# biotite-dev/springcraft

Hardware: AMD Instinct MI355X
Metric: ANM modes/sec (Hessian build + full eigensolve), N=2000 C-alpha (higher is better)
Workload: dtype f64; 1 GPU; C3: N=2000 C-alpha ANM, HinsenForceField (no cutoff), full 6000x6000 eigensolve, all modes + vectors; parallelism=independent structures sharded over GPUs, no data-path collective

## Files before the change

### include/springcraft_hip_debug.h

```cpp
#ifndef SPRINGCRAFT_HIP_DEBUG_H
#define SPRINGCRAFT_HIP_DEBUG_H

#include "springcraft_hip.h"

#ifdef __cplusplus
extern "C" {
#endif

int sc_dbg_gemm_bench(sc_ctx* ctx, int m, int n, int k, int mode, int tile, int split_k, int iters, int beta_one,
                      double* ms_out, double* max_err_out);

int sc_dbg_gemm_host(sc_ctx* ctx, const double* a, const double* b, double* c, int m, int n, int k, int mode, int tile,
                     int split_k, double alpha, double beta, int lower_grid);

int sc_dbg_gemm3_host(sc_ctx* ctx, const double* a, const double* b, double* c, int count, int m, int n, int k, int layout,
                      int lower, double beta);

int sc_dbg_symm3_host(sc_ctx* ctx, const double* a, const double* v, double* x, int count, int m, int split);
int sc_dbg_symm3_stamps(unsigned long long* out4);
int sc_dbg_symm3_bench(sc_ctx* ctx, int count, int m, int split, int iters, double* ms_out);

int sc_dbg_gemm3_bench(sc_ctx* ctx, int count, int m, int n, int k, int layout, int lower, int kernel, int order, int iters,
                       double* ms_out);

int sc_dbg_gemm_stamps(unsigned long long* out4, int reset);

int sc_dbg_gemm_trace(unsigned long long* out, int max_records, int* count, int reset);

int sc_dbg_two_stage(sc_ctx* ctx, const double* a, int n, double* band_out, double* d_out, double* e_out);

int sc_dbg_bt2_stamps(unsigned long long* out);

int sc_dbg_bt2_clock(unsigned long long* out2);

int sc_dbg_bt2_trace(unsigned long long* out);

int sc_dbg_bulge_stamps(unsigned long long* out6);
int sc_dbg_pair_stamps(unsigned long long* out48);
int sc_dbg_chase_stamps(unsigned long long* out16);

int sc_dbg_set_chase(sc_ctx* ctx, int mode, int give_up_after);

int sc_dbg_set_panel_coop(sc_ctx* ctx, int min_rows);
int sc_dbg_set_panel_coop_fail(sc_ctx* ctx, int panel);

int sc_dbg_set_resident(sc_ctx* ctx, int mode, int hook, int workgroups);
// ... 7 lines not shown
```

### springcraft_amd/csrc/gemm_f64.h

```cpp
#pragma once

#include <cstdint>

#include "common.h"

struct GemmDesc {
  const double* a;
  const double* b;
  double* c;
  int m, n, k;
  long long sa_i, sa_k;
  long long sb_k, sb_j;
  long long ldc;
  double alpha, beta;
  const int* a_kidx;
  const int* b_kidx;
  const int* c_jidx;
  int lower_only;
  int row_off, col_off;
  long long split_stride;
  int a_tri;
};

constexpr int kGemmTile = 3;

constexpr int kGemmAmBk = 0, kGemmAkBk = 1, kGemmAmBn = 2;
int launch_gemm_f64(sc_ctx* ctx, const GemmDesc* d_desc, int count, int max_m, int max_n, int tile,
                    int split_k = 1, bool gather = false, bool tri = false, int layout = -1, bool lower_grid = false,
                    int pin_tile = 0);
int gemm_f64_tile(const sc_ctx* ctx, int count, int max_m, int max_n, int layout);

int launch_gemm3_uniform(sc_ctx* ctx, const GemmDesc* d_desc, int count, int m, int n, int k, int layout, int lower,
                         double alpha, double beta, bool aligned16);
bool gemm3_would_take(sc_ctx* ctx, int count, int m, int n, int k, int layout, int lower, double alpha, double beta,
                      bool aligned16);

int launch_symm3(sc_ctx* ctx, const GemmDesc* d_desc, int count, int m, int split, bool aligned16, bool any_size = false);
bool symm3_would_take(sc_ctx* ctx, int count, int m, int split, bool aligned16);
```

### springcraft_amd/csrc/gemm_f64.hip

```cpp
#include <algorithm>
#include <cmath>
#include <cstdlib>
#include <vector>

#include "gemm_f64.h"

namespace {

typedef double d4 __attribute__((ext_vector_type(4)));

template <int X, bool XCONTIG>
struct StageImage {
  static constexpr int kSize = XCONTIG ? 16 * (X + 16) : 8 * (X + 1) * 2;
  __device__ static __forceinline__ int at(int x, int k) {
    return XCONTIG ? k * (X + 16) + x : ((k >> 1) * (X + 1) + x) * 2 + (k & 1);
  }
};

#ifdef GEMM_STAMPS
__device__ unsigned long long g_gemm_stamps[8];
constexpr int kTraceMax = 1 << 16;
__device__ unsigned long long g_gemm_trace[6 * kTraceMax];
__device__ unsigned int g_gemm_trace_n;
#define GEMM_STAMP(var) unsigned long long var; asm volatile("s_memtime %0\n\ts_waitcnt lgkmcnt(0)" : "=s"(var)::"memory");
// ... 231 lines not shown

  GEMM_STAMP(t_loop)
  int buf = 0;
  for (int kt = k_begin; kt < k_end; kt += BK) {
    if (kt + BK < k_end) s_write(buf ^ 1, kt + BK);
    if (kt + 2 * BK < k_end) g_load(kt + 2 * BK);
    const double* a_s = sA + buf * ImgA::kSize + ImgA::at(wm * WM + fr, fk);
    const double* b_s = sB + buf * ImgB::kSize + ImgB::at(wn * WN + fr, fk);
    double af[2][MT], bf[2][NT];
#pragma unroll
    for (int mi = 0; mi < MT; ++mi) af[0][mi] = a_s[ImgA::at(mi * 16, 0)];
#pragma unroll
    for (int ni = 0; ni < NT; ++ni) bf[0][ni] = b_s[ImgB::at(ni * 16, 0)];
#pragma unroll
    for (int k4 = 0; k4 < BK / 4; ++k4) {
      const int cur = k4 & 1, nxt = cur ^ 1;
      if (k4 + 1 < BK / 4) {
#pragma unroll
        for (int mi = 0; mi < MT; ++mi) af[nxt][mi] = a_s[ImgA::at(mi * 16, (k4 + 1) * 4)];
#pragma unroll
        for (int ni = 0; ni < NT; ++ni) bf[nxt][ni] = b_s[ImgB::at(ni * 16, (k4 + 1) * 4)];
      }
#pragma unroll
      for (int ni = 0; ni < NT; ++ni)
#pragma unroll
        for (int mi = 0; mi < MT; ++mi)
          acc[ni][mi] = __builtin_amdgcn_mfma_f64_16x16x4f64(bf[cur][ni], af[cur][mi], acc[ni][mi], 0, 0, 0);
    }
    __syncthreads();
    buf ^= 1;
  }

  GEMM_STAMP(t_epi)
#pragma unroll
  for (int ni = 0; ni < NT; ++ni) {
#pragma unroll
    for (int r = 0; r < 4; ++r) {
      const int col = n0 + wn * WN + ni * 16 + fk + 4 * r;
      if (col >= N) continue;
      gptr ccol = C + (long long)((GATHER && D.c_jidx) ? D.c_jidx[col] : col) * ldc;
#pragma unroll
      for (int mi = 0; mi < MT; ++mi) {
        const int row = m0 + wm * WM + mi * 16 + fr;
        if (row >= M) continue;
        if (lower && (lower2 ? ((row + roff) | 1) : (row + roff)) < (col + coff)) continue;
        ccol[row] = alpha * acc[ni][mi][r];
      }
    }
  }
#ifdef GEMM_STAMPS
  {
    GEMM_STAMP(t_end)
    if (lane == 0) {
      atomicAdd(&g_gemm_stamps[0], t_loop - t_start);
      atomicAdd(&g_gemm_stamps[1], t_epi - t_loop);
      atomicAdd(&g_gemm_stamps[2], t_end - t_epi);
      atomicAdd(&g_gemm_stamps[3], 1ull);
    }
    if (tid == 0) {
      const unsigned slot = atomicAdd(&g_gemm_trace_n, 1u);
      if (slot < (unsigned)kTraceMax) {
        unsigned hwid, xcc;
        asm volatile("s_getreg_b32 %0, hwreg(HW_REG_HW_ID)" : "=s"(hwid));
        asm volatile("s_getreg_b32 %0, hwreg(HW_REG_XCC_ID)" : "=s"(xcc));
        unsigned long long* r = g_gemm_trace + 6ull * slot;
        r[0] = ((unsigned long long)xcc << 32) | hwid;
        r[1] = t_start; r[2] = t_loop; r[3] = t_epi; r[4] = t_end;
        r[5] = blockIdx.x + (unsigned long long)gridDim.x * (blockIdx.y + (unsigned long long)gridDim.y * blockIdx.z);
      }
    }
  }
#endif
}

template <int BM, int BN, bool AM, bool BNC, bool TRI, bool GATHER = false>
void launch_gemm2_inst(hipStream_t st, dim3 grid, const GemmDesc* d_desc, int split_k, bool lower = false) {
  constexpr size_t lds = sizeof(double) * 2 * (size_t)(StageImage<BM, AM>::kSize + StageImage<BN, BNC>::kSize);
  (void)sc_raise_dyn_lds(reinterpret_cast<const void*>(&k_gemm2<BM, BN, AM, BNC, TRI, GATHER>), (int)lds);
  if (lower) {
// ... 225 lines not shown
  D.alpha = alpha; D.beta = beta;
  if (mode == 0) { D.sa_i = 1; D.sa_k = m; D.sb_k = 1; D.sb_j = k; }
  if (mode == 1) { D.sa_i = 1; D.sa_k = m; D.sb_k = n; D.sb_j = 1; D.lower_only = 1; }
  if (mode == 2) { D.sa_i = k; D.sa_k = 1; D.sb_k = 1; D.sb_j = k; }
  D.split_stride = (long long)m * n;
  fail(hipMemcpy(dd, &D, sizeof(D), hipMemcpyHostToDevice));
  if (rc == SC_OK) {
    const int layout = mode == 0 ? kGemmAmBk : (mode == 1 ? kGemmAmBn : kGemmAkBk);
    if (tile < 10 || tile > 13) {
      rc = sc_set_error(ctx, SC_ERR_INVALID_ARG, "tile id %d (10 .. 13)", tile);
    } else {
      g_gemm2_force_tile = tile - 10;
      rc = launch_gemm_f64(ctx, dd, 1, m, n, tile, split_k, false, false, layout, lower_grid != 0);
      g_gemm2_force_tile = 0;
    }
    fail(hipStreamSynchronize(st));
  }
  if (rc == SC_OK) {
    std::vector<double> h(ec);
    fail(hipMemcpy(h.data(), dc, ec * 8, hipMemcpyDeviceToHost));
    if (rc == SC_OK) {
      if (split_k == 1) std::copy(h.begin(), h.end(), c);
      else
        for (size_t i = 0; i < (size_t)m * n; ++i) {
          double sum = 0.0;
          for (int sl = 0; sl < split_k; ++sl) sum += h[(size_t)sl * m * n + i];
          c[i] = sum;
        }
    }
  }
  (void)hipFree(base);
  return rc;
}
```

### springcraft_amd/csrc/sy2sb.hip

```cpp
#include <algorithm>
#include <vector>

#include "twostage_internal.h"

namespace {

constexpr int kEarly = (kIb + 2) / 2;

__global__ __launch_bounds__(256) void k_panel_qr(double* __restrict__ a_all, long long stride_a,
                                                  double* __restrict__ tri_all, TriLayout TL,
                                                  double* __restrict__ sb_all, SbLayout SL, int j0, int j, int nr,
                                                  int c_end) {
  constexpr int LD = kQrRows + 1;
  extern __shared__ __attribute__((aligned(16))) double sm[];
  const int c_lo = j > 0 ? j - 1 : 0;
  const int ncl = c_end - c_lo;
  double* P = sm;
  double* wv = sm + ncl * LD;
  double* vv = wv + kB;
  double* red = vv + kQrRows;
  __shared__ double s_scale, s_beta, s_tau;

  const int n = TL.n;
  const int r0 = j0 + kB, m = n - r0;
// ... 890 lines not shown
      }
      __syncthreads();
    }
    const double tau = s_tau, scale = s_scale;
    for (int c0 = j + 1; c0 < kB; c0 += 8) {
      const int cnt = min(8, kB - c0);
      double a[8] = {0, 0, 0, 0, 0, 0, 0, 0};
      for (int r = j + 1 + tid; r < m; r += 1024) {
        const double x = pj[r];
        for (int i = 0; i < cnt; ++i) a[i] += x * P[(size_t)(c0 + i) * n + r];
      }
      block_sum8(a, cnt);
      if (tid < cnt) s_w[tid] = tau * (P[(size_t)(c0 + tid) * n + j] + scale * a[tid]);
      __syncthreads();
      for (int r = j + tid; r < m; r += 1024) {
        const double v = r > j ? scale * pj[r] : 1.0;
        for (int i = 0; i < cnt; ++i) P[(size_t)(c0 + i) * n + r] -= v * s_w[i];
      }
      __syncthreads();
    }
    for (int r = j + tid; r < m; r += 1024) pj[r] = r > j ? scale * pj[r] : s_beta;
    __syncthreads();
  }
  for (int c = 0; c < kB; ++c)
    for (int r = tid; r < m; r += 1024) {
      const double val = P[(size_t)c * n + r];
      const double v = r > c ? val : (r == c ? 1.0 : 0.0);
      sb[SL.vw + (size_t)c * n + r0 + r] = v;
      sb[SL.wv + (size_t)(kB + c) * n + r0 + r] = -v;
      sb[SL.xv + (size_t)(2 * kB + c) * n + r0 + r] = v;
    }
}

__global__ __launch_bounds__(256) void k_sum_xslices(double* __restrict__ sb_all, SbLayout SL, int r0) {
  const int n = SL.n, p = SL.symm_split;
  double* sb = sb_all + (size_t)blockIdx.z * SL.slab;
  const int which = blockIdx.y / kB, c = blockIdx.y % kB;
  const int r = r0 + blockIdx.x * 256 + threadIdx.x;
  if (r >= n) return;
  const double* src = sb + SL.xsplit + (size_t)which * p * n * kB + (size_t)c * n + r;
  double s = 0.0;
  for (int q = 0; q < p; ++q) s += src[(size_t)q * n * kB];
  sb[SL.xv + (size_t)(which * kB + c) * n + r] = s;
}

__global__ __launch_bounds__(256) void k_sum_p2(double* __restrict__ sb_all, SbLayout SL) {
  double* sb = sb_all + (size_t)blockIdx.y * SL.slab;
  const int i = blockIdx.x * 256 + threadIdx.x;
  double acc = 0.0;
#pragma unroll
  for (int sl = 0; sl < kSmallSplit; ++sl) acc += sb[SL.small2 + (size_t)sl * 2 * kB * kB + i];
  sb[SL.p2 + i] = acc;
}

__global__ __launch_bounds__(1024) void k_sb_small(const double* __restrict__ tri_all, TriLayout TL,
                                                   double* __restrict__ sb_all, SbLayout SL, int j0) {
  constexpr int LD = kB + 1;
  extern __shared__ __attribute__((aligned(16))) double sm[];
  double* G = sm;
  double* M1 = G + kB * LD;
  double* T = M1 + kB * LD;
  double* U = T + kB * LD;
  const double* tri = tri_all + (size_t)blockIdx.x * TL.slab;
  double* sb = sb_all + (size_t)blockIdx.x * SL.slab;
  const int tid = threadIdx.x, nthr = blockDim.x;
  const double* prod = sb + SL.small;
  const size_t slice = (size_t)kB * 3 * kB;
  for (int idx = tid; idx < kB * kB; idx += nthr) {
    const int i = idx & 63, jj = idx >> 6;
    double g = 0.0, x = 0.0;
#pragma unroll
    for (int s = 0; s < kSmallSplit; ++s) {
      const double* ps = prod + s * slice;
      x += ps[i + (size_t)jj * kB] + ps[i + (size_t)(kB + jj) * kB];
      g += ps[i + (size_t)(2 * kB + jj) * kB];
    }
    G[i * LD + jj] = g;
    M1[i * LD + jj] = x;
    T[i * LD + jj] = 0.0;
  }
  __syncthreads();
  if (tid < kB) {
    const int bb = tid >> 4, c = tid & 15, o = bb * 16;
    double x[16];
#pragma unroll
    for (int i = 15; i >= 0; --i) {
      double acc = (i == c) ? 1.0 : 0.0;
#pragma unroll
      for (int l = i + 1; l < 16; ++l) acc -= G[(o + i) * LD + o + l] * x[l];
      x[i] = i <= c ? tri[TL.tau + j0 + o + i] * acc : 0.0;
    }
#pragma unroll
    for (int i = 0; i < 16; ++i) T[(o + i) * LD + o + c] = x[i];
  }
  __syncthreads();
#pragma unroll
  for (int bs = 16; bs <= 32; bs *= 2) {
    const int npair = kB / (2 * bs);
    for (int idx = tid; idx < npair * bs * bs; idx += nthr) {
      const int pr = idx / (bs * bs), e = idx % (bs * bs), i = e / bs, jj = e % bs;
      const int o1 = pr * 2 * bs, o2 = o1 + bs;
      double acc = 0.0;
      for (int l = 0; l <= jj; ++l) acc += G[(o1 + i) * LD + o2 + l] * T[(o2 + l) * LD + o2 + jj];
      U[(o1 + i) * LD + o2 + jj] = acc;
    }
    __syncthreads();
    for (int idx = tid; idx < npair * bs * bs; idx += nthr) {
      const int pr = idx / (bs * bs), e = idx % (bs * bs), i = e / bs, jj = e % bs;
      const int o1 = pr * 2 * bs, o2 = o1 + bs;
      double acc = 0.0;
      for (int l = i; l < bs; ++l) acc += T[(o1 + i) * LD + o1 + l] * U[(o1 + l) * LD + o2 + jj];
      T[(o1 + i) * LD + o2 + jj] = -acc;
    }
    __syncthreads();
  }
  for (int idx = tid; idx < kB * kB; idx += nthr) {
    const int i = idx >> 6, jj = idx & 63;
    double s = 0.0;
    for (int l = 0; l <= jj; ++l) s += M1[i * LD + l] * T[l * LD + jj];
    U[i * LD + jj] = s;
  }
  __syncthreads();
  double* cm = sb + SL.cmat;
  for (int idx = tid; idx < kB * kB; idx += nthr) {
    const int i = idx & 63, jj = idx >> 6;
    double s = 0.0;
    for (int l = 0; l <= i; ++l) s += T[l * LD + i] * U[l * LD + jj];
    const double t = T[i * LD + jj];
    cm[i + (size_t)jj * 3 * kB] = t;
    cm[kB + i + (size_t)jj * 3 * kB] = t;
    cm[2 * kB + i + (size_t)jj * 3 * kB] = -0.5 * s;
  }
}

}


std::vector<GemmDesc> sb_stage1_records(int n, int batch, const std::vector<int>& role, double* d_a, long long stride_a,
                                        double* d_sb_ws, const SbLayout& SL) {
  const sc_host::TwoStageEnv& E = sc_host::two_stage_env();
  const int npanels = (int)role.size();
  std::vector<GemmDesc> h((size_t)npanels * kDescKinds * batch);
  for (int p = 0; p < npanels; ++p) {
    const int j0 = p * kB, r0 = j0 + kB, m = n - r0;
    const int rl = role[(size_t)p];
    const long long vw_w = rl == 2 ? 3 * kB : kB, wv_w = rl == 2 ? 2 * kB : 0;
    for (int b = 0; b < batch; ++b) {
      double* A = d_a + (size_t)b * stride_a;
      double* sb = d_sb_ws + (size_t)b * SL.slab;
      double* a22 = A + (size_t)r0 * n + r0;
      GemmDesc* g = &h[((size_t)p * batch + b) * kDescKinds];
      GemmDesc X1{};
      X1.a = a22; X1.sa_i = 1; X1.sa_k = n; X1.a_tri = 1;
      X1.b = sb + SL.xv + (size_t)2 * kB * n + r0; X1.sb_k = 1; X1.sb_j = n;
      X1.c = sb + SL.xv + r0; X1.ldc = n;
      X1.m = m; X1.n = kB; X1.k = m; X1.alpha = 1.0; X1.beta = 0.0;
      if (SL.symm_split > 1) {
        X1.c = sb + SL.xsplit + r0;
        X1.split_stride = (long long)n * kB;
      }
      g[0] = X1;
      GemmDesc X2 = X1;
      X2.sa_i = n; X2.sa_k = 1; X2.a_tri = 2;
      X2.c = sb + SL.xv + (size_t)kB * n + r0;
      if (SL.symm_split > 1) X2.c = sb + SL.xsplit + (size_t)SL.symm_split * n * kB + r0;
      g[1] = X2;
      GemmDesc P{};
      P.a = sb + SL.xv + (size_t)2 * kB * n + r0; P.sa_i = n; P.sa_k = 1;
      P.b = sb + SL.xv + r0; P.sb_k = 1; P.sb_j = n;
      P.c = sb + SL.small; P.ldc = kB;
      P.m = kB; P.n = 3 * kB; P.k = m; P.alpha = 1.0; P.beta = 0.0;
      P.split_stride = (long long)kB * 3 * kB;
      g[2] = P;
      GemmDesc W{};
      W.a = sb + SL.xv + r0; W.sa_i = 1; W.sa_k = n;
      W.b = sb + SL.cmat; W.sb_k = 1; W.sb_j = 3 * kB;
      W.c = sb + SL.vw + (size_t)vw_w * n + r0; W.ldc = n;
      W.m = m; W.n = kB; W.k = 3 * kB; W.alpha = 1.0; W.beta = 0.0;
      g[3] = W;
      W.c = sb + SL.wv + (size_t)wv_w * n + r0;
      W.alpha = -1.0;
      g[4] = W;
      GemmDesc R{};
      R.a = sb + SL.vw + r0; R.sa_i = 1; R.sa_k = n;
      R.b = sb + SL.wv + r0; R.sb_k = n; R.sb_j = 1;
      R.c = a22; R.ldc = n;
      R.m = m; R.n = m; R.k = rl == 2 ? 4 * kB : 2 * kB; R.alpha = 1.0; R.beta = 1.0;
      R.lower_only = sc_host::symm3_for(E, n) ? 2 : 1;
      g[5] = R;
      GemmDesc D = R;
      D.n = kB; D.k = 2 * kB;
      g[6] = D;
      GemmDesc Q{};
      Q.a = sb + SL.wv + r0; Q.sa_i = n; Q.sa_k = 1;
      Q.b = sb + SL.xv + (size_t)2 * kB * n + r0; Q.sb_k = 1; Q.sb_j = n;
      Q.c = sb + SL.small2; Q.ldc = 2 * kB;
      Q.m = 2 * kB; Q.n = kB; Q.k = m; Q.alpha = 1.0; Q.beta = 0.0;
      Q.split_stride = (long long)2 * kB * kB;
      g[7] = Q;
      GemmDesc Cr{};
      Cr.a = sb + SL.vw + r0; Cr.sa_i = 1; Cr.sa_k = n;
      Cr.b = sb + SL.p2; Cr.sb_k = 1; Cr.sb_j = 2 * kB;
      Cr.c = sb + SL.xv + r0; Cr.ldc = n;
      Cr.m = m; Cr.n = kB; Cr.k = 2 * kB; Cr.alpha = 1.0; Cr.beta = 1.0;
      g[8] = Cr;
    }
  }
  std::vector<GemmDesc> hs(h.size());
  for (int p = 0; p < npanels; ++p)
    for (int b = 0; b < batch; ++b) {
      const GemmDesc* g = &h[((size_t)p * batch + b) * kDescKinds];
      GemmDesc* o = &hs[(size_t)p * kDescKinds * batch];
      for (int kd = 0; kd < kDescKinds; ++kd) o[(size_t)kd * batch + b] = g[kd];
    }
  return hs;
}

struct PanelRun {
  sc_ctx* ctx;
  hipStream_t st;
  double* d_a; long long stride_a; int n, batch;
  double* d_tri_ws; const TriLayout& TL;
  double* d_sb_ws; const SbLayout& SL;
  const GemmDesc* d_descs;
  const std::vector<int>& role;
  sc_host::CoopPlan coop;
  v4i* coop_recs;
  int* coop_ctl;
  bool use_symm3;
  int symm3_nb_min;
  SbTimers& t;
};

static int run_panel(const PanelRun& R, int p, int lo, int hi, hipStream_t ps, bool timed) {
  using sc_host::PanelQr;
  const sc_host::TwoStageEnv& E = sc_host::two_stage_env();
  sc_ctx* ctx = R.ctx;
  const TriLayout& TL = R.TL;
  const SbLayout& SL = R.SL;
  const int n = R.n, batch = R.batch;
  const long long stride_a = R.stride_a;
  struct StreamScope {
    sc_ctx* c; hipStream_t old;
    StreamScope(sc_ctx* c_, hipStream_t s) : c(c_), old(c_->stream) { c->stream = s; }
    ~StreamScope() { c->stream = old; }
  } scope(ctx, ps);
  const int nb = hi - lo;
  const int rl = R.role[(size_t)p];
  double* a_h = R.d_a + (size_t)lo * stride_a;
  double* tri_h = R.d_tri_ws + (size_t)lo * TL.slab;
  double* sb_h = R.d_sb_ws + (size_t)lo * SL.slab;
  const int j0 = p * kB, r0 = j0 + kB, m = n - r0;
  const int nr = std::min(kB, m - 1);
  const int nchunks = (m + kQrRows - 1) / kQrRows;
  const dim3 qgrid((unsigned)nchunks, (unsigned)nb);
  SbLayout SQ = SL;
  if (rl == 2) { SQ.vw += (long long)2 * kB * n; SQ.wv += (long long)2 * kB * n; }
  if (timed) R.t.qr.start();
  const sc_host::PanelQrForm F = sc_host::panel_qr_form(E, R.coop, R.coop_recs != nullptr, m, nb, ps == R.st);
  switch (F.kind) {
    case PanelQr::Coop: {
      const int coop_g = F.coop_g;
      if (p == ctx->coop_fail_panel) SC_HIP(ctx, hipMemsetAsync(R.coop_ctl + 8 * lo, 1, sizeof(int) * 8 * nb, ps));
// ... 18 lines not shown
      constexpr int kW = 512 / 64;
      const size_t lds_wg = sizeof(double) * (size_t)(2 * kW * 8 + 16 + 8 + 8 * kB + kW * kB * 8);
      const dim3 g1((unsigned)nb), b1(512u);
      if (F.ru == 10) hipLaunchKernelGGL((k_panel_wg<10, 1, 512>), g1, b1, lds_wg, ps, a_h, stride_a, tri_h, TL, sb_h, SQ, j0);
      else hipLaunchKernelGGL((k_panel_wg<12, 1, 512>), g1, b1, lds_wg, ps, a_h, stride_a, tri_h, TL, sb_h, SQ, j0);
      break;
    }
    case PanelQr::Blocked: {
      const size_t lds_qr_blk = sizeof(double) * ((size_t)(kIb + 1) * (kQrRows + 1) + kB + kQrRows + 4 * kB);
      const size_t lds_blk_a = sizeof(double) * ((size_t)kB * (kQrRows + 1) + kQrRows + 8 * kB);
      const size_t lds_blk_b = sizeof(double) * ((size_t)kB * (kQrRows + 1) + kIb * kB + 4 * kB);
      hipLaunchKernelGGL(k_panel_qr, qgrid, dim3(256), lds_qr_blk, ps, a_h, stride_a, tri_h, TL, sb_h, SQ, j0, 0, nr, kIb);
      for (int c0 = 0; c0 < kB; c0 += kIb) {
        for (int j = c0 + 1; j < c0 + kIb; ++j)
          hipLaunchKernelGGL(k_panel_qr, qgrid, dim3(256), lds_qr_blk, ps, a_h, stride_a, tri_h, TL, sb_h, SQ, j0, j, nr,
                             c0 + kIb);
        const size_t cut = sizeof(double) * (size_t)c0 * (kQrRows + 1);
        hipLaunchKernelGGL(k_pqr_blk_a, qgrid, dim3(256), lds_blk_a - cut, ps, a_h, stride_a, tri_h, TL, sb_h, SQ, j0, c0);
        if (c0 + kIb < kB)
          hipLaunchKernelGGL(k_pqr_blk_b, qgrid, dim3(256), lds_blk_b - cut, ps, a_h, stride_a, tri_h, TL, sb_h, SQ, j0, c0);
      }
      break;
    }
    case PanelQr::Unblocked: {
      const size_t lds_qr = sizeof(double) * ((size_t)kB * (kQrRows + 1) + kB + kQrRows + 4 * kB);
      for (int j = 0; j <= nr; ++j)
        hipLaunchKernelGGL(k_panel_qr, qgrid, dim3(256), lds_qr, ps, a_h, stride_a, tri_h, TL, sb_h, SQ, j0, j, nr, kB);
      break;
    }
  }
  if (timed) R.t.qr.stop();
  const GemmDesc* g = R.d_descs + (size_t)p * kDescKinds * batch;
  if (timed) R.t.symm.start();
  if (R.use_symm3 && symm3_would_take(ctx, R.symm3_nb_min, m, SL.symm_split, true) &&
      launch_symm3(ctx, g + lo, nb, m, SL.symm_split, true, true) == SC_OK) {
    if (SL.symm_split > 1)
      hipLaunchKernelGGL(k_sum_xslices, dim3((unsigned)((m + 255) / 256), kB, (unsigned)nb), dim3(256), 0, ps, sb_h, SL, r0);
  } else {
    SC_TRY(launch_gemm_f64(ctx, g + lo, nb, m, kB, kGemmTile, SL.symm_split, false, true, kGemmAmBk));
    SC_TRY(launch_gemm_f64(ctx, g + batch + lo, nb, m, kB, kGemmTile, SL.symm_split, false, true, kGemmAkBk));
    if (SL.symm_split > 1)
      hipLaunchKernelGGL(k_sum_xslices, dim3((unsigned)((m + 255) / 256), 2 * kB, (unsigned)nb), dim3(256), 0, ps, sb_h, SL, r0);
  }
  if (rl == 2) {
    SC_TRY(launch_gemm_f64(ctx, g + 7 * batch + lo, nb, 2 * kB, kB, kGemmTile, kSmallSplit, false, false, kGemmAkBk));
    hipLaunchKernelGGL(k_sum_p2, dim3((unsigned)(2 * kB * kB / 256), (unsigned)nb), dim3(256), 0, ps, sb_h, SL);
    SC_TRY(launch_gemm_f64(ctx, g + 8 * batch + lo, nb, m, kB, kGemmTile, 1, false, false, kGemmAmBk));
  }
  if (timed) R.t.symm.stop();
  SC_TRY(launch_gemm_f64(ctx, g + 2 * batch + lo, nb, kB, 3 * kB, kGemmTile, kSmallSplit, false, false, kGemmAkBk));
  const size_t lds_small = sizeof(double) * 4 * kB * (kB + 1);
  hipLaunchKernelGGL(k_sb_small, dim3((unsigned)nb), dim3(1024), lds_small, ps, tri_h, TL, sb_h, SL, j0);
  if (nb == batch) {
    SC_TRY(launch_gemm_f64(ctx, g + 3 * batch, 2 * batch, m, kB, kGemmTile, 1, false, false, kGemmAmBk));
  } else {
    SC_TRY(launch_gemm_f64(ctx, g + 3 * batch + lo, nb, m, kB, kGemmTile, 1, false, false, kGemmAmBk));
    SC_TRY(launch_gemm_f64(ctx, g + 4 * batch + lo, nb, m, kB, kGemmTile, 1, false, false, kGemmAmBk));
  }
  if (timed) R.t.syr2k.start();
  if (rl == 1)
    SC_TRY(launch_gemm_f64(ctx, g + 6 * batch + lo, nb, m, kB, kGemmTile, 1, false, false, kGemmAmBn));
  else
    if (launch_gemm3_uniform(ctx, g + 5 * batch + lo, nb, m, m, rl == 2 ? 4 * kB : 2 * kB, kGemmAmBn, R.use_symm3 ? 2 : 1, 1.0, 1.0,
                             (n & 1) == 0 && (r0 & 1) == 0) != SC_OK)
      SC_TRY(launch_gemm_f64(ctx, g + 5 * batch + lo, nb, m, m, kGemmTile, 1, false, false, kGemmAmBn, true));
  if (timed) R.t.syr2k.stop();
  return SC_OK;
}

int sb_stage1(sc_ctx* ctx, double* d_a, long long stride_a, int n, int batch, double* d_tri_ws, const TriLayout& TL,
              double* d_sb_ws, const SbLayout& SL, const GemmDesc* d_descs, const std::vector<int>& role, bool prof,
              SbTimers& timers) {
  const sc_host::TwoStageEnv& E = sc_host::two_stage_env();
  hipStream_t st = ctx->stream;
  const int npanels = (int)role.size();

  for (int b = 0; b < batch; ++b)
    SC_HIP(ctx, hipMemsetAsync(d_tri_ws + (size_t)b * TL.slab + TL.tau, 0, sizeof(double) * n, st));

  const int s1_parts = sc_host::stage1_parts(E, batch, prof);
  const sc_host::CoopPlan coop = sc_host::coop_plan(E, n, batch, ctx->num_cus, prof, ctx->coop_min_rows, ctx->coop_ok);
  v4i* coop_recs = nullptr;
  int* coop_ctl = nullptr;
  if (coop.ask) {
    if (ctx->coop_attr < 0)
      ctx->coop_attr = hipFuncSetAttribute(reinterpret_cast<const void*>(&k_panel_coop),
                                           hipFuncAttributeMaxDynamicSharedMemorySize, (int)kCoopLdsBytes) == hipSuccess;
    if (ctx->coop_attr == 1 && coop.nb_max >= 1) {
      const size_t rec_bytes = (size_t)batch * coop_recs_per_matrix(coop.gmax) * sizeof(v4i);
      const size_t ctl_bytes = align_up((size_t)batch * 8 * sizeof(int), 256);
      SC_TRY(sc_reserve_dc_aux(ctx, ctl_bytes + rec_bytes));
      coop_ctl = reinterpret_cast<int*>(ctx->dc_aux);
      coop_recs = reinterpret_cast<v4i*>(reinterpret_cast<char*>(ctx->dc_aux) + ctl_bytes);
      SC_HIP(ctx, hipMemsetAsync(ctx->dc_aux, 0, ctl_bytes + rec_bytes, st));
    }
  }
  const bool use_symm3 = sc_host::symm3_for(E, n);
  if (use_symm3)
    for (int b = 0; b < batch; ++b)
      SC_HIP(ctx, hipMemsetAsync(d_sb_ws + (size_t)b * SL.slab + SL.xv + (size_t)kB * n, 0, sizeof(double) * (size_t)kB * n, st));
  const PanelRun R{ctx, st, d_a, stride_a, n, batch, d_tri_ws, TL, d_sb_ws, SL, d_descs, role, coop, coop_recs, coop_ctl,
                   use_symm3, std::max(1, batch / s1_parts), timers};
  if (s1_parts > 1) {
    struct SideBySide {
      sc_ctx* c;
      explicit SideBySide(sc_ctx* c_) : c(c_) { c->gemm3_side_by_side = true; }
      ~SideBySide() { c->gemm3_side_by_side = false; }
    } side_by_side(ctx);
    SC_TRY(sc_aux_stream(ctx));
    SC_TRY(sc_side_streams(ctx, s1_parts - 1));
    SC_HIP(ctx, hipEventRecord(ctx->aux_fork, st));
    for (int q = 1; q < s1_parts; ++q) SC_HIP(ctx, hipStreamWaitEvent(ctx->side_streams[q - 1], ctx->aux_fork, 0));
    int rc_parts = SC_OK;
    for (int p = 0; p < npanels && rc_parts == SC_OK; ++p)
      for (int q = 0; q < s1_parts && rc_parts == SC_OK; ++q) {
        const int lo = (int)((long long)batch * q / s1_parts), hi = (int)((long long)batch * (q + 1) / s1_parts);
        rc_parts = run_panel(R, p, lo, hi, q == 0 ? st : ctx->side_streams[q - 1], q == 0);
      }
    for (int q = 1; q < s1_parts; ++q) {
      SC_HIP(ctx, hipEventRecord(ctx->side_joins[q - 1], ctx->side_streams[q - 1]));
      SC_HIP(ctx, hipStreamWaitEvent(st, ctx->side_joins[q - 1], 0));
    }
    SC_TRY(rc_parts);
  } else {
    for (int p = 0; p < npanels; ++p) SC_TRY(run_panel(R, p, 0, batch, st, true));
  }
  SC_HIP(ctx, hipGetLastError());
  return SC_OK;
}
```

### springcraft_amd/csrc/twostage.hip

```cpp
#include <algorithm>
#include <vector>

#include "twostage_internal.h"

size_t sb_slab_doubles(int n, int batch, SbLayout* out) {
  SbLayout L{};
  L.n = n;
  long long off = 0;
  auto take = [&](long long cnt) { long long o = off; off += (cnt + 31) / 32 * 32; return o; };
  const int nchunk = (n + kQrRows - 1) / kQrRows + 1;
  L.vw = take((long long)n * 4 * kB);
  L.wv = take((long long)n * 4 * kB);
  L.xv = take((long long)n * 3 * kB);
  L.symm_split = sc_host::symm_split_for(sc_host::two_stage_env(), n, batch);
  L.xsplit = L.symm_split > 1 ? take((long long)2 * L.symm_split * n * kB) : 0;
  L.qrpart = take((long long)2 * nchunk * kB);
  L.qrpiv = take(2 * (kB + 8));
  L.qrpart8 = take((long long)nchunk * kIb * kB);
  L.small = take((long long)kSmallSplit * kB * 3 * kB);
  L.cmat = take(3 * kB * kB);
  L.small2 = take((long long)kSmallSplit * 2 * kB * kB);
  L.p2 = take(2 * kB * kB);
  L.ab = take((long long)kLdab * n);
  const int nsweep = std::max(n - 2, 0);
  L.ngroups = (nsweep + kG - 1) / kG;
  long long ndia = 0;
  for (int S = 0; S < L.ngroups; ++S) {
    const int len = (n - 1 - S * kG + kB - 1) / kB;
    ndia += len;
  }
  L.ndia = ndia;
  L.vd = take(ndia * kDiaSize);
  L.frag = take(ndia * kFragDoubles);
  L.tau2 = take(ndia * kG);
  L.slab = off;
  if (out) *out = L;
  return (size_t)off;
}

int sb_desc_count(int n, int batch) {
  const int npanels = n / kB + 1;
  return npanels * kDescKinds * batch;
}

int sytrd_2stage_batched(sc_ctx* ctx, double* d_a, long long stride_a, int n, int batch, double* d_tri_ws,
                         const TriLayout& TL, double* d_sb_ws, const SbLayout& SL, int* d_dia_off,
                         GemmDesc* d_descs, float* ms_stage1, float* ms_stage2, double* d_band_copy) {
  hipStream_t st = ctx->stream;
  ScopedEvents<3> ev;
  const bool prof = ctx->profiling && ms_stage1 && ms_stage2;
  if (prof) {
    for (auto& e : ev) SC_HIP(ctx, hipEventCreate(&e));
    SC_HIP(ctx, hipEventRecord(ev[0], st));
  }

  const std::vector<int> role = sc_host::panel_roles(sc_host::two_stage_env(), n);
  const std::vector<GemmDesc> hs = sb_stage1_records(n, batch, role, d_a, stride_a, d_sb_ws, SL);
  if (!hs.empty()) SC_TRY(sc_stage_upload(ctx, d_descs, hs.data(), hs.size() * sizeof(GemmDesc)));
  const std::vector<int> doff = dia_offsets(n);
  SC_TRY(sc_stage_upload(ctx, d_dia_off, doff.data(), doff.size() * sizeof(int)));

  SbTimers timers(ctx, st);
  SC_TRY(sb_stage1(ctx, d_a, stride_a, n, batch, d_tri_ws, TL, d_sb_ws, SL, d_descs, role, prof, timers));
  if (prof) SC_HIP(ctx, hipEventRecord(ev[1], st));
  SC_TRY(sb_stage2(ctx, d_a, stride_a, n, batch, d_tri_ws, TL, d_sb_ws, SL, d_band_copy, timers));
  if (prof) {
    SC_HIP(ctx, hipEventRecord(ev[2], st));
    SC_HIP(ctx, hipEventSynchronize(ev[2]));
    SC_HIP(ctx, hipEventElapsedTime(ms_stage1, ev[0], ev[1]));
    SC_HIP(ctx, hipEventElapsedTime(ms_stage2, ev[1], ev[2]));
  }
  timers.finish();
  return SC_OK;
}

int sb_band_width() { return kB; }

extern "C" int sc_dbg_two_stage(sc_ctx* ctx, const double* a, int n, double* band_out, double* d_out, double* e_out) {
  if (!ctx || !a || n < 4 * kB) return SC_ERR_INVALID_ARG;
  SC_HIP(ctx, hipSetDevice(ctx->device));
  TriLayout TL{};
  TL.n = n; TL.nb = kB;
  TL.d = 0; TL.e = n; TL.tau = 2 * (long long)n; TL.slab = 3 * (long long)n + 64;
  SbLayout SL;
  const size_t sbd = sb_slab_doubles(n, 1, &SL);
  double *d_a = nullptr, *d_tri = nullptr, *d_sb = nullptr, *d_band = nullptr;
  int* d_off = nullptr;
  GemmDesc* d_desc = nullptr;
  SC_HIP(ctx, hipMalloc(&d_a, sizeof(double) * (size_t)n * n));
  SC_HIP(ctx, hipMalloc(&d_tri, sizeof(double) * TL.slab));
  SC_HIP(ctx, hipMalloc(&d_sb, sizeof(double) * sbd));
  SC_HIP(ctx, hipMalloc(&d_band, sizeof(double) * kLdab * n));
  SC_HIP(ctx, hipMalloc(&d_off, sizeof(int) * (n / 64 + 8)));
  SC_HIP(ctx, hipMalloc(&d_desc, sizeof(GemmDesc) * sb_desc_count(n, 1)));
  SC_HIP(ctx, hipMemcpyAsync(d_a, a, sizeof(double) * (size_t)n * n, hipMemcpyHostToDevice, ctx->stream));
  int rc = mirror_lower_batched(ctx, d_a, (long long)n * n, n, 1);
  if (rc == SC_OK)
    rc = sytrd_2stage_batched(ctx, d_a, (long long)n * n, n, 1, d_tri, TL, d_sb, SL, d_off, d_desc, nullptr, nullptr,
                              d_band);
  if (rc == SC_OK) {
    (void)hipMemcpy(band_out, d_band, sizeof(double) * kLdab * n, hipMemcpyDeviceToHost);
    (void)hipMemcpy(d_out, d_tri + TL.d, sizeof(double) * n, hipMemcpyDeviceToHost);
    (void)hipMemcpy(e_out, d_tri + TL.e, sizeof(double) * n, hipMemcpyDeviceToHost);
  }
  (void)hipFree(d_a); (void)hipFree(d_tri); (void)hipFree(d_sb); (void)hipFree(d_band); (void)hipFree(d_off);
  (void)hipFree(d_desc);
  return rc;
}
```

### springcraft_amd/csrc/twostage_internal.h

```cpp
#pragma once

#include <algorithm>
#include <vector>

#include "eigh_internal.h"
#include "twostage_policy.h"

namespace {

constexpr int kB = sc_host::kBand;
constexpr int kG = 64;
constexpr int kDiaLd = 128;
constexpr int kDiaSize = kDiaLd * kG;

constexpr int kMiniFrags = 40;
constexpr int kDiaFrags = 4 * kMiniFrags;
constexpr int kFragDoubles = kDiaFrags * 64;

constexpr int kLdab = 2 * kB;
constexpr int kQrRows = 128;
constexpr int kSmallSplit = 8;
constexpr int kDescKinds = 9;
#ifndef SC_QR_IB
#define SC_QR_IB 8
#endif
constexpr int kIb = SC_QR_IB;

typedef int v4i __attribute__((ext_vector_type(4)));

struct HH {
  double beta, tau, scale;
};

__device__ __forceinline__ HH householder(double alpha, double xn2) {
  HH h;
  if (xn2 == 0.0 || alpha * alpha + xn2 < 1e-280) {
    h.beta = alpha; h.tau = 0.0; h.scale = 0.0;
    return h;
  }
  h.beta = -copysign(sqrt(alpha * alpha + xn2), alpha);
  h.tau = (h.beta - alpha) / h.beta;
  h.scale = 1.0 / (alpha - h.beta);
  return h;
}

__device__ __forceinline__ void lds_barrier() { asm volatile("s_waitcnt lgkmcnt(0)\n\ts_barrier" ::: "memory"); }

__device__ __forceinline__ double wave_sum(double v) {
#pragma unroll
  for (int off = 32; off > 0; off >>= 1) v += __shfl_xor(v, off);
  return v;
}

typedef double __attribute__((address_space(1)))* gdptr;
__device__ __forceinline__ gdptr wave_uniform(double* p) {
  const unsigned long long b = (unsigned long long)(size_t)p;
  const unsigned lo = (unsigned)__builtin_amdgcn_readfirstlane((int)(unsigned)b);
  const unsigned hi = (unsigned)__builtin_amdgcn_readfirstlane((int)(unsigned)(b >> 32));
  return (gdptr)(size_t)(((unsigned long long)hi << 32) | (unsigned long long)lo);
}

}

inline std::vector<int> dia_offsets(int n) {
  const int nsweep = std::max(n - 2, 0);
  const int ng = (nsweep + kG - 1) / kG;
  std::vector<int> off((size_t)ng + 1, 0);
  for (int S = 0; S < ng; ++S) off[(size_t)S + 1] = off[(size_t)S] + (n - 1 - S * kG + kB - 1) / kB;
  return off;
}

struct SbTimers {
  PhaseTimer qr, symm, syr2k, bulge;
  SbTimers(sc_ctx* ctx, hipStream_t st) : qr(ctx, "panel_qr", st), symm(ctx, "symm", st), syr2k(ctx, "syr2k", st), bulge(ctx, "bulge", st) {}
  void finish() { qr.finish(); symm.finish(); syr2k.finish(); bulge.finish(); }
};

std::vector<GemmDesc> sb_stage1_records(int n, int batch, const std::vector<int>& role, double* d_a, long long stride_a,
                                        double* d_sb_ws, const SbLayout& SL);
int sb_stage1(sc_ctx* ctx, double* d_a, long long stride_a, int n, int batch, double* d_tri_ws, const TriLayout& TL,
              double* d_sb_ws, const SbLayout& SL, const GemmDesc* d_descs, const std::vector<int>& role, bool prof,
              SbTimers& timers);
int sb_stage2(sc_ctx* ctx, double* d_a, long long stride_a, int n, int batch, double* d_tri_ws, const TriLayout& TL,
              double* d_sb_ws, const SbLayout& SL, double* d_band_copy, SbTimers& timers);
```

Baseline: 180,900 modes/s.

## Fuse W/-W GEMMs via negated epilogue and shrink X blocks when symm3 takes

The GEMM epilogue can now also write the negated result to a second output, so the separate W and -W GEMM launches per panel collapse into one. When the symmetric symm3 kernel handles a panel, X is written as a single block at an offset, which lets the small product and cmat use two blocks instead of three and removes the per-batch zeroing memsets. The per-batch tau memsets are replaced by a single zeroing kernel. This cuts GEMM launches, some FLOPs in the small products, and memset overhead. The cost is extra epilogue stores and a hard error when symm3 declines a panel that was pre-planned to use it.

```diff
diff --git a/include/springcraft_hip_debug.h b/include/springcraft_hip_debug.h
--- a/include/springcraft_hip_debug.h
+++ b/include/springcraft_hip_debug.h
@@ -12,6 +12,9 @@
 
 int sc_dbg_gemm_host(sc_ctx* ctx, const double* a, const double* b, double* c, int m, int n, int k, int mode, int tile,
                      int split_k, double alpha, double beta, int lower_grid);
+
+int sc_dbg_gemm_neg_host(sc_ctx* ctx, const double* a, const double* b, double* c, double* cneg, int m, int n, int k,
+                         int tile, double alpha, double beta, int ldn, int use_neg);
 
 int sc_dbg_gemm3_host(sc_ctx* ctx, const double* a, const double* b, double* c, int count, int m, int n, int k, int layout,
                       int lower, double beta);
diff --git a/springcraft_amd/csrc/gemm_f64.h b/springcraft_amd/csrc/gemm_f64.h
--- a/springcraft_amd/csrc/gemm_f64.h
+++ b/springcraft_amd/csrc/gemm_f64.h
@@ -20,6 +20,8 @@
   int row_off, col_off;
   long long split_stride;
   int a_tri;
+  double* c_neg;
+  long long ldc_neg;
 };
 
 constexpr int kGemmTile = 3;
diff --git a/springcraft_amd/csrc/gemm_f64.hip b/springcraft_amd/csrc/gemm_f64.hip
--- a/springcraft_amd/csrc/gemm_f64.hip
+++ b/springcraft_amd/csrc/gemm_f64.hip
@@ -287,6 +287,8 @@
   }
 
   GEMM_STAMP(t_epi)
+  const gptr Cn = (GATHER || split_k > 1) ? (gptr) nullptr : (gptr)D.c_neg;
+  const long long ldc_neg = D.ldc_neg;
 #pragma unroll
   for (int ni = 0; ni < NT; ++ni) {
 #pragma unroll
@@ -294,12 +296,15 @@
       const int col = n0 + wn * WN + ni * 16 + fk + 4 * r;
       if (col >= N) continue;
       gptr ccol = C + (long long)((GATHER && D.c_jidx) ? D.c_jidx[col] : col) * ldc;
+      gptr ncol = Cn + (long long)col * ldc_neg;
 #pragma unroll
       for (int mi = 0; mi < MT; ++mi) {
         const int row = m0 + wm * WM + mi * 16 + fr;
         if (row >= M) continue;
         if (lower && (lower2 ? ((row + roff) | 1) : (row + roff)) < (col + coff)) continue;
-        ccol[row] = alpha * acc[ni][mi][r];
+        const double val = alpha * acc[ni][mi][r];
+        ccol[row] = val;
+        if (Cn) ncol[row] = -val;
       }
     }
   }
@@ -591,3 +596,42 @@
   (void)hipFree(base);
   return rc;
 }
+
+extern "C" int sc_dbg_gemm_neg_host(sc_ctx* ctx, const double* a, const double* b, double* c, double* cneg, int m, int n,
+                                    int k, int tile, double alpha, double beta, int ldn, int use_neg) {
+  if (!ctx || !a || !b || !c || !cneg || m <= 0 || n <= 0 || k <= 0 || ldn < m) return SC_ERR_INVALID_ARG;
+  if (tile < 10 || tile > 13) return sc_set_error(ctx, SC_ERR_INVALID_ARG, "tile id %d (10 .. 13)", tile);
+  SC_HIP(ctx, hipSetDevice(ctx->device));
+  const size_t ea = (size_t)m * k, eb = (size_t)k * n, ec = (size_t)m * n, en = (size_t)ldn * n;
+  char* base = nullptr;
+  SC_HIP(ctx, hipMalloc((void**)&base, (ea + eb + ec + en) * 8 + 256));
+  double* da = (double*)base;
+  double* db = da + ea;
+  double* dc = db + eb;
+  double* dn = dc + ec;
+  GemmDesc* dd = (GemmDesc*)(dn + en);
+  int rc = SC_OK;
+  auto fail = [&](hipError_t e) { if (e != hipSuccess && rc == SC_OK) rc = sc_set_error(ctx, SC_ERR_HIP, "%s", hipGetErrorString(e)); };
+  fail(hipMemcpy(da, a, ea * 8, hipMemcpyHostToDevice));
+  fail(hipMemcpy(db, b, eb * 8, hipMemcpyHostToDevice));
+  fail(hipMemcpy(dc, c, ec * 8, hipMemcpyHostToDevice));
+  fail(hipMemcpy(dn, cneg, en * 8, hipMemcpyHostToDevice));
+  GemmDesc D{};
+  D.a = da; D.b = db; D.c = dc; D.m = m; D.n = n; D.k = k; D.ldc = m;
+  D.alpha = alpha; D.beta = beta;
+  D.sa_i = 1; D.sa_k = m; D.sb_k = 1; D.sb_j = k;
+  if (use_neg) { D.c_neg = dn; D.ldc_neg = ldn; }
+  fail(hipMemcpy(dd, &D, sizeof(D), hipMemcpyHostToDevice));
+  if (rc == SC_OK) {
+    g_gemm2_force_tile = tile - 10;
+    rc = launch_gemm_f64(ctx, dd, 1, m, n, tile, 1, false, false, kGemmAmBk);
+    g_gemm2_force_tile = 0;
+    fail(hipStreamSynchronize(ctx->stream));
+  }
+  if (rc == SC_OK) {
+    fail(hipMemcpy(c, dc, ec * 8, hipMemcpyDeviceToHost));
+    fail(hipMemcpy(cneg, dn, en * 8, hipMemcpyDeviceToHost));
+  }
+  (void)hipFree(base);
+  return rc;
+}
diff --git a/springcraft_amd/csrc/sy2sb.hip b/springcraft_amd/csrc/sy2sb.hip
--- a/springcraft_amd/csrc/sy2sb.hip
+++ b/springcraft_amd/csrc/sy2sb.hip
@@ -946,7 +946,7 @@
     }
 }
 
-__global__ __launch_bounds__(256) void k_sum_xslices(double* __restrict__ sb_all, SbLayout SL, int r0) {
+__global__ __launch_bounds__(256) void k_sum_xslices(double* __restrict__ sb_all, SbLayout SL, int r0, int dst_col) {
   const int n = SL.n, p = SL.symm_split;
   double* sb = sb_all + (size_t)blockIdx.z * SL.slab;
   const int which = blockIdx.y / kB, c = blockIdx.y % kB;
@@ -955,7 +955,7 @@
   const double* src = sb + SL.xsplit + (size_t)which * p * n * kB + (size_t)c * n + r;
   double s = 0.0;
   for (int q = 0; q < p; ++q) s += src[(size_t)q * n * kB];
-  sb[SL.xv + (size_t)(which * kB + c) * n + r] = s;
+  sb[SL.xv + (size_t)(dst_col + which * kB + c) * n + r] = s;
 }
 
 __global__ __launch_bounds__(256) void k_sum_p2(double* __restrict__ sb_all, SbLayout SL) {
@@ -967,8 +967,13 @@
   sb[SL.p2 + i] = acc;
 }
 
+__global__ __launch_bounds__(256) void k_zero_tau(double* __restrict__ tri_all, TriLayout TL) {
+  const int i = blockIdx.x * 256 + threadIdx.x;
+  if (i < TL.n) tri_all[(size_t)blockIdx.y * TL.slab + TL.tau + i] = 0.0;
+}
+
 __global__ __launch_bounds__(1024) void k_sb_small(const double* __restrict__ tri_all, TriLayout TL,
-                                                   double* __restrict__ sb_all, SbLayout SL, int j0) {
+                                                   double* __restrict__ sb_all, SbLayout SL, int j0, int two_block) {
   constexpr int LD = kB + 1;
   extern __shared__ __attribute__((aligned(16))) double sm[];
   double* G = sm;
@@ -978,16 +983,17 @@
   const double* tri = tri_all + (size_t)blockIdx.x * TL.slab;
   double* sb = sb_all + (size_t)blockIdx.x * SL.slab;
   const int tid = threadIdx.x, nthr = blockDim.x;
+  const int nblk = two_block ? 2 : 3;
   const double* prod = sb + SL.small;
-  const size_t slice = (size_t)kB * 3 * kB;
+  const size_t slice = (size_t)kB * nblk * kB;
   for (int idx = tid; idx < kB * kB; idx += nthr) {
     const int i = idx & 63, jj = idx >> 6;
     double g = 0.0, x = 0.0;
 #pragma unroll
     for (int s = 0; s < kSmallSplit; ++s) {
       const double* ps = prod + s * slice;
-      x += ps[i + (size_t)jj * kB] + ps[i + (size_t)(kB + jj) * kB];
-      g += ps[i + (size_t)(2 * kB + jj) * kB];
+      x += two_block ? ps[i + (size_t)jj * kB] : ps[i + (size_t)jj * kB] + ps[i + (size_t)(kB + jj) * kB];
+      g += ps[i + (size_t)((nblk - 1) * kB + jj) * kB];
     }
     G[i * LD + jj] = g;
     M1[i * LD + jj] = x;
@@ -1036,22 +1042,34 @@
   }
   __syncthreads();
   double* cm = sb + SL.cmat;
+  const size_t ldcm = (size_t)nblk * kB;
   for (int idx = tid; idx < kB * kB; idx += nthr) {
     const int i = idx & 63, jj = idx >> 6;
     double s = 0.0;
     for (int l = 0; l <= i; ++l) s += T[l * LD + i] * U[l * LD + jj];
     const double t = T[i * LD + jj];
-    cm[i + (size_t)jj * 3 * kB] = t;
-    cm[kB + i + (size_t)jj * 3 * kB] = t;
-    cm[2 * kB + i + (size_t)jj * 3 * kB] = -0.5 * s;
-  }
-}
-
-}
-
-
-std::vector<GemmDesc> sb_stage1_records(int n, int batch, const std::vector<int>& role, double* d_a, long long stride_a,
-                                        double* d_sb_ws, const SbLayout& SL) {
+    cm[i + jj * ldcm] = t;
+    if (!two_block) cm[kB + i + jj * ldcm] = t;
+    cm[(nblk - 1) * kB + i + jj * ldcm] = -0.5 * s;
+  }
+}
+
+}
+
+
+std::vector<char> sb_stage1_two_block(sc_ctx* ctx, int n, int batch, const SbLayout& SL, bool prof) {
+  const sc_host::TwoStageEnv& E = sc_host::two_stage_env();
+  const int npanels = sc_host::panel_count(n);
+  std::vector<char> two((size_t)npanels, 0);
+  if (!sc_host::symm3_for(E, n)) return two;
+  const int nb_min = std::max(1, batch / sc_host::stage1_parts(E, batch, prof));
+  for (int p = 0; p < npanels; ++p)
+    two[(size_t)p] = symm3_would_take(ctx, nb_min, n - (p + 1) * kB, SL.symm_split, true);
+  return two;
+}
+
+std::vector<GemmDesc> sb_stage1_records(int n, int batch, const std::vector<int>& role, const std::vector<char>& two_block,
+                                        double* d_a, long long stride_a, double* d_sb_ws, const SbLayout& SL) {
   const sc_host::TwoStageEnv& E = sc_host::two_stage_env();
   const int npanels = (int)role.size();
   std::vector<GemmDesc> h((size_t)npanels * kDescKinds * batch);
@@ -1059,6 +1077,9 @@
     const int j0 = p * kB, r0 = j0 + kB, m = n - r0;
     const int rl = role[(size_t)p];
     const long long vw_w = rl == 2 ? 3 * kB : kB, wv_w = rl == 2 ? 2 * kB : 0;
+    const bool two = two_block[(size_t)p] != 0;
+    const int nblk = two ? 2 : 3;
+    const size_t xoff = two ? (size_t)kB * n : 0;
     for (int b = 0; b < batch; ++b) {
       double* A = d_a + (size_t)b * stride_a;
       double* sb = d_sb_ws + (size_t)b * SL.slab;
@@ -1067,7 +1088,7 @@
       GemmDesc X1{};
       X1.a = a22; X1.sa_i = 1; X1.sa_k = n; X1.a_tri = 1;
       X1.b = sb + SL.xv + (size_t)2 * kB * n + r0; X1.sb_k = 1; X1.sb_j = n;
-      X1.c = sb + SL.xv + r0; X1.ldc = n;
+      X1.c = sb + SL.xv + xoff + r0; X1.ldc = n;
       X1.m = m; X1.n = kB; X1.k = m; X1.alpha = 1.0; X1.beta = 0.0;
       if (SL.symm_split > 1) {
         X1.c = sb + SL.xsplit + r0;
@@ -1081,43 +1102,41 @@
       g[1] = X2;
       GemmDesc P{};
       P.a = sb + SL.xv + (size_t)2 * kB * n + r0; P.sa_i = n; P.sa_k = 1;
-      P.b = sb + SL.xv + r0; P.sb_k = 1; P.sb_j = n;
+      P.b = sb + SL.xv + xoff + r0; P.sb_k = 1; P.sb_j = n;
       P.c = sb + SL.small; P.ldc = kB;
-      P.m = kB; P.n = 3 * kB; P.k = m; P.alpha = 1.0; P.beta = 0.0;
-      P.split_stride = (long long)kB * 3 * kB;
+      P.m = kB; P.n = nblk * kB; P.k = m; P.alpha = 1.0; P.beta = 0.0;
+      P.split_stride = (long long)kB * nblk * kB;
       g[2] = P;
       GemmDesc W{};
-      W.a = sb + SL.xv + r0; W.sa_i = 1; W.sa_k = n;
-      W.b = sb + SL.cmat; W.sb_k = 1; W.sb_j = 3 * kB;
+      W.a = sb + SL.xv + xoff + r0; W.sa_i = 1; W.sa_k = n;
+      W.b = sb + SL.cmat; W.sb_k = 1; W.sb_j = nblk * kB;
       W.c = sb + SL.vw + (size_t)vw_w * n + r0; W.ldc = n;
-      W.m = m; W.n = kB; W.k = 3 * kB; W.alpha = 1.0; W.beta = 0.0;
+      W.c_neg = sb + SL.wv + (size_t)wv_w * n + r0; W.ldc_neg = n;
+      W.m = m; W.n = kB; W.k = nblk * kB; W.alpha = 1.0; W.beta = 0.0;
       g[3] = W;
-      W.c = sb + SL.wv + (size_t)wv_w * n + r0;
-      W.alpha = -1.0;
-      g[4] = W;
       GemmDesc R{};
       R.a = sb + SL.vw + r0; R.sa_i = 1; R.sa_k = n;
       R.b = sb + SL.wv + r0; R.sb_k = n; R.sb_j = 1;
       R.c = a22; R.ldc = n;
       R.m = m; R.n = m; R.k = rl == 2 ? 4 * kB : 2 * kB; R.alpha = 1.0; R.beta = 1.0;
       R.lower_only = sc_host::symm3_for(E, n) ? 2 : 1;
-      g[5] = R;
+      g[4] = R;
       GemmDesc D = R;
       D.n = kB; D.k = 2 * kB;
-      g[6] = D;
+      g[5] = D;
       GemmDesc Q{};
       Q.a = sb + SL.wv + r0; Q.sa_i = n; Q.sa_k = 1;
       Q.b = sb + SL.xv + (size_t)2 * kB * n + r0; Q.sb_k = 1; Q.sb_j = n;
       Q.c = sb + SL.small2; Q.ldc = 2 * kB;
       Q.m = 2 * kB; Q.n = kB; Q.k = m; Q.alpha = 1.0; Q.beta = 0.0;
       Q.split_stride = (long long)2 * kB * kB;
-      g[7] = Q;
+      g[6] = Q;
       GemmDesc Cr{};
       Cr.a = sb + SL.vw + r0; Cr.sa_i = 1; Cr.sa_k = n;
       Cr.b = sb + SL.p2; Cr.sb_k = 1; Cr.sb_j = 2 * kB;
-      Cr.c = sb + SL.xv + r0; Cr.ldc = n;
+      Cr.c = sb + SL.xv + xoff + r0; Cr.ldc = n;
       Cr.m = m; Cr.n = kB; Cr.k = 2 * kB; Cr.alpha = 1.0; Cr.beta = 1.0;
-      g[8] = Cr;
+      g[7] = Cr;
     }
   }
   std::vector<GemmDesc> hs(h.size());
@@ -1138,11 +1157,11 @@
   double* d_sb_ws; const SbLayout& SL;
   const GemmDesc* d_descs;
   const std::vector<int>& role;
+  const std::vector<char>& two_block;
   sc_host::CoopPlan coop;
   v4i* coop_recs;
   int* coop_ctl;
   bool use_symm3;
-  int symm3_nb_min;
   SbTimers& t;
 };
 
@@ -1227,51 +1246,47 @@
   if (timed) R.t.qr.stop();
   const GemmDesc* g = R.d_descs + (size_t)p * kDescKinds * batch;
   if (timed) R.t.symm.start();
-  if (R.use_symm3 && symm3_would_take(ctx, R.symm3_nb_min, m, SL.symm_split, true) &&
-      launch_symm3(ctx, g + lo, nb, m, SL.symm_split, true, true) == SC_OK) {
+  const bool two = R.two_block[(size_t)p] != 0;
+  if (two) {
+    if (launch_symm3(ctx, g + lo, nb, m, SL.symm_split, true, true) != SC_OK)
+      return sc_set_error(ctx, SC_ERR_HIP, "band reduction: k_symm3 did not take panel %d (m = %d, %d matrices)", p, m, nb);
     if (SL.symm_split > 1)
-      hipLaunchKernelGGL(k_sum_xslices, dim3((unsigned)((m + 255) / 256), kB, (unsigned)nb), dim3(256), 0, ps, sb_h, SL, r0);
+      hipLaunchKernelGGL(k_sum_xslices, dim3((unsigned)((m + 255) / 256), kB, (unsigned)nb), dim3(256), 0, ps, sb_h, SL, r0, kB);
   } else {
     SC_TRY(launch_gemm_f64(ctx, g + lo, nb, m, kB, kGemmTile, SL.symm_split, false, true, kGemmAmBk));
     SC_TRY(launch_gemm_f64(ctx, g + batch + lo, nb, m, kB, kGemmTile, SL.symm_split, false, true, kGemmAkBk));
     if (SL.symm_split > 1)
-      hipLaunchKernelGGL(k_sum_xslices, dim3((unsigned)((m + 255) / 256), 2 * kB, (unsigned)nb), dim3(256), 0, ps, sb_h, SL, r0);
+      hipLaunchKernelGGL(k_sum_xslices, dim3((unsigned)((m + 255) / 256), 2 * kB, (unsigned)nb), dim3(256), 0, ps, sb_h, SL, r0, 0);
   }
   if (rl == 2) {
-    SC_TRY(launch_gemm_f64(ctx, g + 7 * batch + lo, nb, 2 * kB, kB, kGemmTile, kSmallSplit, false, false, kGemmAkBk));
+    SC_TRY(launch_gemm_f64(ctx, g + 6 * batch + lo, nb, 2 * kB, kB, kGemmTile, kSmallSplit, false, false, kGemmAkBk));
     hipLaunchKernelGGL(k_sum_p2, dim3((unsigned)(2 * kB * kB / 256), (unsigned)nb), dim3(256), 0, ps, sb_h, SL);
-    SC_TRY(launch_gemm_f64(ctx, g + 8 * batch + lo, nb, m, kB, kGemmTile, 1, false, false, kGemmAmBk));
+    SC_TRY(launch_gemm_f64(ctx, g + 7 * batch + lo, nb, m, kB, kGemmTile, 1, false, false, kGemmAmBk));
   }
   if (timed) R.t.symm.stop();
-  SC_TRY(launch_gemm_f64(ctx, g + 2 * batch + lo, nb, kB, 3 * kB, kGemmTile, kSmallSplit, false, false, kGemmAkBk));
+  SC_TRY(launch_gemm_f64(ctx, g + 2 * batch + lo, nb, kB, (two ? 2 : 3) * kB, kGemmTile, kSmallSplit, false, false, kGemmAkBk));
   const size_t lds_small = sizeof(double) * 4 * kB * (kB + 1);
-  hipLaunchKernelGGL(k_sb_small, dim3((unsigned)nb), dim3(1024), lds_small, ps, tri_h, TL, sb_h, SL, j0);
-  if (nb == batch) {
-    SC_TRY(launch_gemm_f64(ctx, g + 3 * batch, 2 * batch, m, kB, kGemmTile, 1, false, false, kGemmAmBk));
-  } else {
-    SC_TRY(launch_gemm_f64(ctx, g + 3 * batch + lo, nb, m, kB, kGemmTile, 1, false, false, kGemmAmBk));
-    SC_TRY(launch_gemm_f64(ctx, g + 4 * batch + lo, nb, m, kB, kGemmTile, 1, false, false, kGemmAmBk));
-  }
+  hipLaunchKernelGGL(k_sb_small, dim3((unsigned)nb), dim3(1024), lds_small, ps, tri_h, TL, sb_h, SL, j0, two ? 1 : 0);
+  SC_TRY(launch_gemm_f64(ctx, g + 3 * batch + lo, nb, m, kB, kGemmTile, 1, false, false, kGemmAmBk));
   if (timed) R.t.syr2k.start();
   if (rl == 1)
-    SC_TRY(launch_gemm_f64(ctx, g + 6 * batch + lo, nb, m, kB, kGemmTile, 1, false, false, kGemmAmBn));
+    SC_TRY(launch_gemm_f64(ctx, g + 5 * batch + lo, nb, m, kB, kGemmTile, 1, false, false, kGemmAmBn));
   else
-    if (launch_gemm3_uniform(ctx, g + 5 * batch + lo, nb, m, m, rl == 2 ? 4 * kB : 2 * kB, kGemmAmBn, R.use_symm3 ? 2 : 1, 1.0, 1.0,
+    if (launch_gemm3_uniform(ctx, g + 4 * batch + lo, nb, m, m, rl == 2 ? 4 * kB : 2 * kB, kGemmAmBn, R.use_symm3 ? 2 : 1, 1.0, 1.0,
                              (n & 1) == 0 && (r0 & 1) == 0) != SC_OK)
-      SC_TRY(launch_gemm_f64(ctx, g + 5 * batch + lo, nb, m, m, kGemmTile, 1, false, false, kGemmAmBn, true));
+      SC_TRY(launch_gemm_f64(ctx, g + 4 * batch + lo, nb, m, m, kGemmTile, 1, false, false, kGemmAmBn, true));
   if (timed) R.t.syr2k.stop();
   return SC_OK;
 }
 
 int sb_stage1(sc_ctx* ctx, double* d_a, long long stride_a, int n, int batch, double* d_tri_ws, const TriLayout& TL,
-              double* d_sb_ws, const SbLayout& SL, const GemmDesc* d_descs, const std::vector<int>& role, bool prof,
-              SbTimers& timers) {
+              double* d_sb_ws, const SbLayout& SL, const GemmDesc* d_descs, const std::vector<int>& role,
+              const std::vector<char>& two_block, bool prof, SbTimers& timers) {
   const sc_host::TwoStageEnv& E = sc_host::two_stage_env();
   hipStream_t st = ctx->stream;
   const int npanels = (int)role.size();
 
-  for (int b = 0; b < batch; ++b)
-    SC_HIP(ctx, hipMemsetAsync(d_tri_ws + (size_t)b * TL.slab + TL.tau, 0, sizeof(double) * n, st));
+  hipLaunchKernelGGL(k_zero_tau, dim3((unsigned)((n + 255) / 256), (unsigned)batch), dim3(256), 0, st, d_tri_ws, TL);
 
   const int s1_parts = sc_host::stage1_parts(E, batch, prof);
   const sc_host::CoopPlan coop = sc_host::coop_plan(E, n, batch, ctx->num_cus, prof, ctx->coop_min_rows, ctx->coop_ok);
@@ -1291,11 +1306,8 @@
     }
   }
   const bool use_symm3 = sc_host::symm3_for(E, n);
-  if (use_symm3)
-    for (int b = 0; b < batch; ++b)
-      SC_HIP(ctx, hipMemsetAsync(d_sb_ws + (size_t)b * SL.slab + SL.xv + (size_t)kB * n, 0, sizeof(double) * (size_t)kB * n, st));
-  const PanelRun R{ctx, st, d_a, stride_a, n, batch, d_tri_ws, TL, d_sb_ws, SL, d_descs, role, coop, coop_recs, coop_ctl,
-                   use_symm3, std::max(1, batch / s1_parts), timers};
+  const PanelRun R{ctx, st, d_a, stride_a, n, batch, d_tri_ws, TL, d_sb_ws, SL, d_descs, role, two_block, coop, coop_recs,
+                   coop_ctl, use_symm3, timers};
   if (s1_parts > 1) {
     struct SideBySide {
       sc_ctx* c;
diff --git a/springcraft_amd/csrc/twostage.hip b/springcraft_amd/csrc/twostage.hip
--- a/springcraft_amd/csrc/twostage.hip
+++ b/springcraft_amd/csrc/twostage.hip
@@ -55,13 +55,14 @@
   }
 
   const std::vector<int> role = sc_host::panel_roles(sc_host::two_stage_env(), n);
-  const std::vector<GemmDesc> hs = sb_stage1_records(n, batch, role, d_a, stride_a, d_sb_ws, SL);
+  const std::vector<char> two_block = sb_stage1_two_block(ctx, n, batch, SL, prof);
+  const std::vector<GemmDesc> hs = sb_stage1_records(n, batch, role, two_block, d_a, stride_a, d_sb_ws, SL);
   if (!hs.empty()) SC_TRY(sc_stage_upload(ctx, d_descs, hs.data(), hs.size() * sizeof(GemmDesc)));
   const std::vector<int> doff = dia_offsets(n);
   SC_TRY(sc_stage_upload(ctx, d_dia_off, doff.data(), doff.size() * sizeof(int)));
 
   SbTimers timers(ctx, st);
-  SC_TRY(sb_stage1(ctx, d_a, stride_a, n, batch, d_tri_ws, TL, d_sb_ws, SL, d_descs, role, prof, timers));
+  SC_TRY(sb_stage1(ctx, d_a, stride_a, n, batch, d_tri_ws, TL, d_sb_ws, SL, d_descs, role, two_block, prof, timers));
   if (prof) SC_HIP(ctx, hipEventRecord(ev[1], st));
   SC_TRY(sb_stage2(ctx, d_a, stride_a, n, batch, d_tri_ws, TL, d_sb_ws, SL, d_band_copy, timers));
   if (prof) {
@@ -98,6 +99,7 @@
   if (rc == SC_OK)
     rc = sytrd_2stage_batched(ctx, d_a, (long long)n * n, n, 1, d_tri, TL, d_sb, SL, d_off, d_desc, nullptr, nullptr,
                               d_band);
+  if (rc == SC_OK && hipStreamSynchronize(ctx->stream) != hipSuccess) rc = sc_set_error(ctx, SC_ERR_HIP, "two-stage debug solve failed");
   if (rc == SC_OK) {
     (void)hipMemcpy(band_out, d_band, sizeof(double) * kLdab * n, hipMemcpyDeviceToHost);
     (void)hipMemcpy(d_out, d_tri + TL.d, sizeof(double) * n, hipMemcpyDeviceToHost);
diff --git a/springcraft_amd/csrc/twostage_internal.h b/springcraft_amd/csrc/twostage_internal.h
--- a/springcraft_amd/csrc/twostage_internal.h
+++ b/springcraft_amd/csrc/twostage_internal.h
@@ -20,7 +20,7 @@
 constexpr int kLdab = 2 * kB;
 constexpr int kQrRows = 128;
 constexpr int kSmallSplit = 8;
-constexpr int kDescKinds = 9;
+constexpr int kDescKinds = 8;
 #ifndef SC_QR_IB
 #define SC_QR_IB 8
 #endif
@@ -76,10 +76,11 @@
   void finish() { qr.finish(); symm.finish(); syr2k.finish(); bulge.finish(); }
 };
 
-std::vector<GemmDesc> sb_stage1_records(int n, int batch, const std::vector<int>& role, double* d_a, long long stride_a,
-                                        double* d_sb_ws, const SbLayout& SL);
+std::vector<char> sb_stage1_two_block(sc_ctx* ctx, int n, int batch, const SbLayout& SL, bool prof);
+std::vector<GemmDesc> sb_stage1_records(int n, int batch, const std::vector<int>& role, const std::vector<char>& two_block,
+                                        double* d_a, long long stride_a, double* d_sb_ws, const SbLayout& SL);
 int sb_stage1(sc_ctx* ctx, double* d_a, long long stride_a, int n, int batch, double* d_tri_ws, const TriLayout& TL,
-              double* d_sb_ws, const SbLayout& SL, const GemmDesc* d_descs, const std::vector<int>& role, bool prof,
-              SbTimers& timers);
+              double* d_sb_ws, const SbLayout& SL, const GemmDesc* d_descs, const std::vector<int>& role,
+              const std::vector<char>& two_block, bool prof, SbTimers& timers);
 int sb_stage2(sc_ctx* ctx, double* d_a, long long stride_a, int n, int batch, double* d_tri_ws, const TriLayout& TL,
               double* d_sb_ws, const SbLayout& SL, double* d_band_copy, SbTimers& timers);
```

Result: no change. 180,700 modes/s (-0.1%).
